# distributed-information-bottleneck/distributed-information-bottleneck.github.io

Measured on AMD Instinct MI355X. Metric: DIB train samples/sec (fwd+KL+bwd+Adam), higher is better.
Workload: dtype f32; 1 GPU; BASELINE config 3: synthetic tabular, 2^20 rows x 64 scalar features resident in HBM, posenc [2,4,8,16], encoder [128,128], E=32, integration [256,256], out=1, BCE-from-logits, Adam; per_gpu_batch=65536, global_batch=65536, parallelism=dp1, rccl_ranks_joined=1, dataset_rows=1048576, params=2224897

## Files before the change

### distributed-information-bottleneck.github.io_amd/_lib.py

```python
from __future__ import annotations

import ctypes
import os
import shutil
import subprocess
from ctypes import POINTER, c_char_p, c_float, c_int, c_int32, c_int64, c_uint32, c_uint64, c_void_p

_HERE = os.path.dirname(os.path.abspath(__file__))
CSRC = os.path.join(_HERE, "csrc")
LIB_PATH = os.path.join(_HERE, "libdib_hip.so")
LIB_OVERRIDE = os.environ.get("DIB_LIB_PATH") or None
INCLUDE_DIR = os.path.join(os.path.dirname(_HERE), "include")


def _sources() -> list:
    out = []
    for root, _, names in os.walk(CSRC):
        out += [os.path.join(root, n) for n in names if n.endswith((".h", ".hip"))]
    out += [os.path.join(INCLUDE_DIR, n) for n in os.listdir(INCLUDE_DIR) if n.endswith(".h")]
    return sorted(out)


DIB_OK = 0
ABI_VERSION = 7
# ... 85 lines not shown
    "dib_get_tuning": (c_int, [c_char_p, POINTER(c_int)]),
    "dib_adam_step": (c_int, [c_void_p, c_void_p, c_void_p, c_void_p, c_int64, c_void_p, c_void_p, c_float, c_float,
                              c_float, c_float, c_void_p]),
    "dib_sgd_step": (c_int, [c_void_p, c_void_p, c_int64, c_void_p, c_float, c_void_p]),
    "dib_encode_deterministic": (c_int, [c_void_p, c_int, c_void_p, c_int, c_void_p, c_void_p, c_void_p, c_void_p]),
    "dib_bhattacharyya": (c_int, [c_void_p, c_void_p, c_int, c_void_p, c_void_p, c_int, c_int, c_void_p, c_void_p]),
    "dib_infonce_workspace_bytes": (c_int64, [c_int]),
    "dib_infonce_fwd_bwd": (c_int, [c_void_p, c_void_p, c_int, c_int, c_int, c_float, c_void_p, c_void_p, c_void_p, c_void_p,
                                    c_void_p]),
    "dib_positional_encoding": (c_int, [c_void_p, c_int64, c_int, c_int, c_int, c_void_p, c_void_p]),
    "dib_positional_encoding_rows": (c_int, [c_void_p, c_int64, c_void_p, c_int, c_int, c_int, c_void_p, c_void_p]),
    "dib_mlp_small_supported": (c_int, [c_void_p, c_int]),
    "dib_mlp_small_fwd": (c_int, [c_void_p, c_void_p, c_void_p, c_int64, c_void_p, c_int, c_void_p, c_void_p, c_void_p, c_void_p]),
    "dib_mlp_small_bwd": (c_int, [c_void_p, c_void_p, c_void_p, c_void_p, c_void_p, c_int, c_void_p]),
    "dib_mlp_small_head_supported": (c_int, [c_void_p, c_int]),
    "dib_mlp_small_head_workspace_bytes": (c_int64, [c_void_p, c_int]),
    "dib_mlp_small_head_step": (c_int, [c_void_p, c_void_p, c_void_p, c_int, c_void_p, c_int64, c_int, c_float, c_void_p, c_void_p,
                                        c_void_p, c_void_p, c_void_p, c_void_p, c_void_p, c_void_p, c_void_p]),
    "dib_integration_fwd_and_mlp_fwd": (c_int, [c_void_p, c_int, c_void_p, c_void_p, c_void_p, c_void_p, c_void_p, c_int64, c_void_p,
                                                c_int, c_void_p, c_void_p, c_void_p, c_void_p]),
    "dib_backward_and_mlp_bwd": (c_int, [c_void_p, c_int, c_void_p, c_void_p, c_void_p, c_float, c_int, c_void_p, c_void_p, c_void_p,
                                         c_void_p, c_void_p, c_void_p, c_int, c_void_p]),
    "dib_reduce_adam_step": (c_int, [c_void_p, c_int, c_int64, c_void_p, c_void_p, c_void_p, c_void_p, c_int64, c_void_p, c_void_p,
                                     c_float, c_float, c_float, c_float, c_void_p, c_void_p]),
    "dib_mi_workspace_bytes": (c_int64, [c_int, c_int]),
    "dib_mi_sandwich_rows": (c_int, [c_void_p, c_int, c_int, c_uint64, c_uint32, c_uint32, c_void_p, c_void_p, c_void_p,
                                     c_void_p]),
    "dib_philox_normal_fill": (c_int, [c_void_p, c_void_p, c_int64, c_int, c_int, c_int, c_uint64, c_uint32,
                                       c_void_p]),
    "dib_philox_normal_ref": (c_float, [c_uint64, c_uint32, c_uint32, c_uint32, c_uint32]),
    "dib_launch_count": (c_int64, []),
    "dib_profile_enable": (c_int, [c_int]),
    "dib_profile_summary": (c_int, [POINTER(ctypes.c_double), POINTER(c_int)]),
    "dib_gemm": (c_int, [c_int, c_int, c_int, c_int, c_void_p, c_int, c_void_p, c_int, c_void_p, c_int, c_void_p,
                         c_void_p, c_int, c_int, c_void_p, c_void_p]),
}

SIGNATURES_ST = {
    "dib_gemm_grouped": (c_int, [c_int, c_int, c_void_p, c_int, c_int, c_void_p, c_void_p, c_void_p, c_void_p, c_void_p,
                                 c_void_p, c_int, c_int, c_int, c_int64, c_void_p]),
    "dib_reduce_splits": (c_int, [c_void_p, c_int64, c_int, c_int64, c_void_p, c_void_p]),
    "dib_reduce_splits_add": (c_int, [c_void_p, c_int64, c_int, c_int64, c_void_p, c_void_p]),
    "dib_gemm_skinny_k": (c_int, [c_int, c_int, c_void_p, c_int, c_int, c_int, c_void_p, c_void_p, c_void_p, c_void_p, c_void_p]),
    "dib_softmax_rows_fwd": (c_int, [c_void_p, c_int64, c_int, c_int, c_float, c_void_p]),
    "dib_softmax_rows_bwd": (c_int, [c_void_p, c_void_p, c_int64, c_int, c_int, c_float, c_void_p]),
    "dib_attention_stash_bytes": (c_int64, [c_int, c_int, c_int]),
    "dib_attention_fwd": (c_int, [c_void_p, c_void_p, c_void_p, c_int, c_int, c_int, c_int, c_int64, c_float, c_void_p, c_void_p,
                                  c_void_p, c_void_p]),
    "dib_attention_fwd_proj_supported": (c_int, [c_int, c_int, c_int]),
    "dib_attention_fwd_proj": (c_int, [c_void_p, c_int64, c_void_p, c_void_p, c_void_p, c_int, c_int, c_int, c_int, c_int, c_int64, c_float,
                                       c_void_p, c_void_p, c_void_p, c_void_p, c_void_p, c_void_p]),
    "dib_attention_bwd_proj": (c_int, [c_void_p, c_void_p, c_void_p, c_void_p, c_void_p, c_int, c_int, c_int, c_int, c_int, c_int64, c_float,
                                       c_void_p, c_void_p, c_void_p, c_void_p, c_void_p, c_void_p, c_int64, c_void_p]),
    "dib_attention_bwd_workspace_bytes": (c_int64, [c_int, c_int, c_int]),
    "dib_attention_bwd": (c_int, [c_void_p, c_void_p, c_void_p, c_void_p, c_void_p, c_void_p, c_void_p, c_int, c_int, c_int, c_int,
                                  c_int64, c_float, c_void_p, c_void_p, c_void_p, c_void_p, c_void_p]),
    "dib_add_layernorm_fwd": (c_int, [c_void_p, c_void_p, c_int, c_int64, c_int64, c_int, c_void_p, c_void_p, c_float, c_void_p,
                                      c_void_p, c_void_p, c_void_p]),
    "dib_add_layernorm_bwd_workspace_bytes": (c_int64, [c_int64, c_int]),
    "dib_add_layernorm_bwd": (c_int, [c_void_p, c_void_p, c_void_p, c_void_p, c_int64, c_int, c_void_p, c_void_p, c_void_p,
                                      c_void_p]),
    "dib_add_layernorm_bwd_fused": (c_int, [c_void_p, c_void_p, c_void_p, c_void_p, c_void_p, c_int64, c_int, c_void_p, c_void_p,
                                            c_int, c_void_p, c_void_p, c_void_p, c_void_p]),
    "dib_st_chain_supported": (c_int, [c_void_p, c_int64]),
    "dib_st_chain_workspace_bytes": (c_int64, [c_int64, c_int]),
    "dib_st_chain_fwd": (c_int, [c_void_p, c_int64, c_void_p, c_void_p, c_void_p, c_void_p, c_void_p, c_void_p, c_void_p, c_void_p,
                                 c_void_p, c_void_p, c_void_p]),
    "dib_st_chain_bwd": (c_int, [c_void_p, c_int64, c_void_p, c_void_p, c_int, c_int64, c_void_p, c_void_p, c_void_p, c_void_p, c_void_p,
                                 c_void_p, c_void_p, c_void_p, c_void_p, c_void_p, c_void_p]),
    "dib_mean_pool_fwd": (c_int, [c_void_p, c_int, c_int, c_int, c_void_p, c_void_p]),
    "dib_mean_pool_bwd": (c_int, [c_void_p, c_int, c_int, c_int, c_void_p, c_void_p]),
    "dib_add_inplace": (c_int, [c_void_p, c_void_p, c_int64, c_void_p]),
    "dib_act_grad_mul": (c_int, [c_void_p, c_void_p, c_int, c_int64, c_void_p, c_void_p]),
# ... 110 lines not shown
```

### distributed-information-bottleneck.github.io_amd/csrc/dib_api.hip

```cpp
#include <algorithm>
#include <atomic>
#include <cmath>
#include <cstdio>
#include <cstdlib>
#include <cstring>
#include <map>
#include <mutex>
#include <new>
#include <utility>
#include <vector>

#include "../../include/dib_hip.h"
#include "dib_elementwise.h"
#include "dib_gauss_lse.h"
#include "dib_mi_rows.h"
#include "dib_gemm.h"
#include "dib_infonce_mfma.h"
#include "dib_fused.h"
#include "dib_tail.h"
#include "dib_small.h"
#include "dib_st.h"
#include "dib_attn.h"
#include "dib_attn_small.h"
#include "dib_st_chain.h"
#include "dib_measure.h"
#include "dib_circuit.h"
#include "dib_partition.h"
#include "dib_st_info.h"
#include "dib_mi_channel.h"
#include "../../include/dib_st.h"
#include "../../include/dib_measure.h"
#include "../../include/dib_circuit.h"
#include "../../include/dib_partition.h"
#include "../../include/dib_mi_channel.h"

#include "host/common.h"
#include "host/layout.h"
#include "host/gemm.h"
#include "host/encoder.h"
#include "host/small.h"
#include "host/step.h"
#include "host/infonce.h"
#include "host/st.h"
#include "host/mi.h"
#include "host/measure.h"
#include "host/circuit.h"
#include "host/partition.h"
```

### distributed-information-bottleneck.github.io_amd/csrc/host/common.h

```cpp

static std::atomic<unsigned long long> g_dib_launches{0};
#define DIB_LAUNCH(...) do { g_dib_launches.fetch_add(1, std::memory_order_relaxed); hipLaunchKernelGGL(__VA_ARGS__); } while (0)

namespace {

constexpr int64_t kAlign = 64;
constexpr int kMaxSplits = 32;
constexpr int kSmallMaxBatch = 2048;
constexpr int kSmallMaxEncWgs = 1024;
constexpr size_t kSmallMaxLds = 160 * 1024;
constexpr int kSplitRows = 512;
inline int64_t align_up(int64_t v, int64_t a = kAlign) { return (v + a - 1) / a * a; }
inline int cdiv(int64_t a, int64_t b) { return (int)((a + b - 1) / b); }
inline int grid_for(int64_t n, int per_block = 256, int cap = 256 * 16) {
  return (int)std::max<int64_t>(1, std::min<int64_t>((n + per_block - 1) / per_block, cap));
}

constexpr int kProfCats = 17;
constexpr int kProfFusedFwd = 12, kProfFusedBwd = 13, kProfOther = 14, kProfAttnFwd = 15, kProfAttnBwd = 16;
struct Prof {
  std::atomic<bool> on{false};
  std::mutex mu;
  std::vector<hipEvent_t> pool;
  std::vector<std::pair<hipEvent_t, hipEvent_t>> spans[kProfCats];
  hipEvent_t get() {
    if (!pool.empty()) { hipEvent_t e = pool.back(); pool.pop_back(); return e; }
    hipEvent_t e = nullptr;
    (void)hipEventCreate(&e);
    return e;
  }
} g_prof;

struct ProfScope {
  int cat; hipStream_t st; hipEvent_t a = nullptr, b = nullptr;
  ProfScope(int c, hipStream_t s) : cat(c), st(s) {
    if (g_prof.on.load(std::memory_order_relaxed) && cat != 14) {
      { std::lock_guard<std::mutex> lk(g_prof.mu); a = g_prof.get(); b = g_prof.get(); }
      (void)hipEventRecord(a, st);
    }
  }
  ~ProfScope() {
    if (a) { (void)hipEventRecord(b, st); std::lock_guard<std::mutex> lk(g_prof.mu); g_prof.spans[cat].push_back({a, b}); }
  }
};

const char* kVersion = "dib_hip 0.4 (gfx950: fused encoder-bank fwd/bwd + grouped fp32-MFMA GEMM + flash attention)";

int act_ok(int a) { return a >= 0 && a <= 7; }

struct Tuning {
  int fwd_small_wgs = 512;
  int fwd_narrow_wgs = 1024;
  int stream_rows = 8192;
  int split_policy = 1;
  int split_overhead = 128;
  int fused_encoder = 1;
  int fused_head = 1;
  int small_batch = 1;
  int small_wgs = 512;
  int mlp_row_tiles = 1;
  int infonce_one_launch = 1;
  int attn_small_bwd_waves = 8;
  int wgrad_flat_tile = 1;
  int attn_fwd_waves = 8;
  int int_cluster_short_exchange = 1;
  int int_cluster = 8;
  int int_cluster_wgs = 256;
  int int_cluster_min_weights = 65536;
  int wgrad_max_splits = 32;
  int num_cus = 0;
};
inline Tuning& tuning() { static Tuning t; return t; }
inline const Tuning& knobs() { return tuning(); }
inline int wgrad_max_splits() { return std::max(1, std::min(32, knobs().wgrad_max_splits)); }
inline int device_cus() {
  static std::atomic<int> cus[64];
  int dev = 0;
  if (hipGetDevice(&dev) != hipSuccess || dev < 0 || dev >= 64) return 256;
  int v = cus[dev].load(std::memory_order_relaxed);
  if (v > 0) return v;
  if (hipDeviceGetAttribute(&v, hipDeviceAttributeMultiprocessorCount, dev) != hipSuccess || v <= 0) return 256;
  cus[dev].store(v, std::memory_order_relaxed);
  return v;
}
inline int split_rule_cus() { return knobs().num_cus > 0 ? knobs().num_cus : device_cus(); }

std::mutex g_attr_mu;
template <auto* Kernel>
int raise_dynamic_lds(size_t bytes) {
  if (bytes <= 64 * 1024) return DIB_OK;
  static std::atomic<size_t> granted[64];
  int dev = 0;
  std::atomic<size_t>* slot = hipGetDevice(&dev) == hipSuccess && dev >= 0 && dev < 64 ? &granted[dev] : nullptr;
  if (slot && slot->load(std::memory_order_acquire) >= bytes) return DIB_OK;
  std::lock_guard<std::mutex> lk(g_attr_mu);
  if (slot && slot->load(std::memory_order_relaxed) >= bytes) return DIB_OK;
  hipError_t e = hipFuncSetAttribute((const void*)Kernel, hipFuncAttributeMaxDynamicSharedMemorySize, (int)bytes);
  if (e != hipSuccess) return (int)e;
  if (slot) slot->store(bytes, std::memory_order_release);
  return DIB_OK;
}
template <auto* Kernel, typename... Args>
int launch_lds(dim3 grid, dim3 block, size_t lds, hipStream_t st, Args&&... args) {
  if (int rc = raise_dynamic_lds<Kernel>(lds)) return rc;
  DIB_LAUNCH(Kernel, grid, block, lds, st, std::forward<Args>(args)...);
  return (int)hipGetLastError();
}

static int* tuning_slot(const char* key) {
  Tuning& t = tuning();
  if (!key) return nullptr;
  if (!std::strcmp(key, "fwd_small_wgs")) return &t.fwd_small_wgs;
  if (!std::strcmp(key, "fwd_narrow_wgs")) return &t.fwd_narrow_wgs;
  if (!std::strcmp(key, "stream_rows")) return &t.stream_rows;
  if (!std::strcmp(key, "split_policy")) return &t.split_policy;
  if (!std::strcmp(key, "split_overhead")) return &t.split_overhead;
  if (!std::strcmp(key, "fused_encoder")) return &t.fused_encoder;
  if (!std::strcmp(key, "fused_head")) return &t.fused_head;
  if (!std::strcmp(key, "small_batch")) return &t.small_batch;
  if (!std::strcmp(key, "small_wgs")) return &t.small_wgs;
  if (!std::strcmp(key, "mlp_row_tiles")) return &t.mlp_row_tiles;
  if (!std::strcmp(key, "infonce_one_launch")) return &t.infonce_one_launch;
  if (!std::strcmp(key, "attn_small_bwd_waves")) return &t.attn_small_bwd_waves;
  if (!std::strcmp(key, "wgrad_flat_tile")) return &t.wgrad_flat_tile;
  if (!std::strcmp(key, "wgrad_max_splits")) return &t.wgrad_max_splits;
  if (!std::strcmp(key, "num_cus")) return &t.num_cus;
  if (!std::strcmp(key, "attn_fwd_waves")) return &t.attn_fwd_waves;
  if (!std::strcmp(key, "int_cluster_short_exchange")) return &t.int_cluster_short_exchange;
  if (!std::strcmp(key, "int_cluster")) return &t.int_cluster;
  if (!std::strcmp(key, "int_cluster_wgs")) return &t.int_cluster_wgs;
  if (!std::strcmp(key, "int_cluster_min_weights")) return &t.int_cluster_min_weights;
  return nullptr;
}

}

extern "C" {

const char* dib_version(void) { return kVersion; }
int dib_abi_version(void) { return DIB_ABI_VERSION; }

const char* dib_error_string(int code) {
  switch (code) {
    case DIB_OK: return "ok";
    case DIB_E_ARG: return "invalid argument";
    case DIB_E_SHAPE: return "shape mismatch";
    case DIB_E_WORKSPACE: return "workspace / descriptor tables missing";
    case DIB_E_UNSUPPORTED: return "unsupported configuration";
    case DIB_E_NODEVICE: return "no HIP device";
    default: return code > 0 ? hipGetErrorString((hipError_t)code) : "unknown dib error";
  }
}

int dib_set_tuning(const char* key, int value) {
  int* p = tuning_slot(key);
  if (!p || value < 0) return DIB_E_ARG;
  *p = value;
  return DIB_OK;
}

int dib_get_tuning(const char* key, int* value) {
  const int* p = tuning_slot(key);
  if (!p || !value) return DIB_E_ARG;
  *value = *p;
  return DIB_OK;
}

int64_t dib_launch_count(void) { return (int64_t)g_dib_launches.load(std::memory_order_relaxed); }

int dib_profile_enable(int on) {
  std::lock_guard<std::mutex> lk(g_prof.mu);
  for (int c = 0; c < kProfCats; ++c) {
    for (auto& sp : g_prof.spans[c]) { g_prof.pool.push_back(sp.first); g_prof.pool.push_back(sp.second); }
    g_prof.spans[c].clear();
  }
  g_prof.on = on != 0;
  return DIB_OK;
}

int dib_profile_summary(double* ms_by_category, int* launches_by_category) {
  if (!ms_by_category || !launches_by_category) return DIB_E_ARG;
  std::lock_guard<std::mutex> lk(g_prof.mu);
  for (int c = 0; c < kProfCats; ++c) {
    double tot = 0.0;
    for (auto& sp : g_prof.spans[c]) {
      hipError_t e = hipEventSynchronize(sp.second);
      if (e != hipSuccess) return (int)e;
      float ms = 0.f;
      e = hipEventElapsedTime(&ms, sp.first, sp.second);
      if (e != hipSuccess) return (int)e;
      tot += ms;
    }
    ms_by_category[c] = tot;
    launches_by_category[c] = (int)g_prof.spans[c].size();
  }
  return DIB_OK;
}

}
```

### distributed-information-bottleneck.github.io_amd/csrc/host/gemm.h

```cpp

namespace {

template <int MODE, int NI, int NJ, bool FLAT = false>
int launch_gemm_t(const DibGemmGroup* dev_groups, const GemmCall& c, int M, int N, const float* A, const float* B, float* C,
                  const float* bias, const float* aux, float* bias_out, int batch, int act, int nsplit,
                  int rows_per_split, long long split_stride, hipStream_t st) {
  const int tm = cdiv(M, FLAT ? 32 : 64 * NI), tn = cdiv(N, FLAT ? 256 : 64 * NJ);
  if (c.count > 65535 || (MODE == 2 && (long long)tm * tn > 65535)) return DIB_E_UNSUPPORTED;
  dim3 grid;
  if (MODE == 2) grid = dim3(nsplit, tm * tn, c.count);
  else grid = dim3(8 * cdiv(tm, 8) * tn, 1, c.count);
  constexpr int BK = FLAT ? 32 : ((NI == 2 && NJ == 2) ? 64 : ((MODE == 2 && NI == 1 && NJ == 2) ? 64 : 32));
  const long long streamed_rows = MODE == 2 ? (long long)nsplit * rows_per_split : (long long)M;
  const bool big_out = MODE != 2 && (long long)M * N * (long long)sizeof(float) * c.count >= (256ll << 20);
  const int stream_flags = streamed_rows >= knobs().stream_rows ? (big_out ? 3 : 1) : 0;
  DIB_LAUNCH((dib_gemm_kernel<MODE, NI, NJ, BK, FLAT>), grid, dim3(256), 0, st, dev_groups + c.first, A, B, C,
                     bias, aux, bias_out, batch, act, tm, tn, rows_per_split, split_stride, stream_flags);
  return (int)hipGetLastError();
}

static void pick_wgrad_splits(long long tiles, int slots, int K, int max_splits, int* ns_out, int* rps_out) {
  const int min_rows = std::min(kSplitRows, std::max(64, *rps_out));
  const auto cost_of = [&](int ns, int rps) {
    return (double)((tiles * ns + slots - 1) / slots) * (rps + knobs().split_overhead);
  };
  {
    const long long wgs = tiles * *ns_out, rounds = (wgs + slots - 1) / slots;
    if ((double)wgs >= 0.85 * (double)(rounds * slots)) return;
  }
  double best = 1e300;
  int bns = *ns_out, brps = *rps_out;
  for (int ns = 1; ns <= max_splits; ++ns) {
    const int rps = cdiv(cdiv(K, ns), 64) * 64;
    if (ns > 1 && rps < min_rows) break;
    if (cdiv(K, rps) != ns) continue;
    const double cost = cost_of(ns, rps);
    if (cost < best) {
      best = cost;
      bns = ns;
      brps = rps;
    }
  }
  if (best >= cost_of(*ns_out, *rps_out)) return;
  *ns_out = bns;
  *rps_out = brps;
}

template <int MODE>
int launch_gemm(const DibGemmGroup* dev_groups, const GemmCall& c, const float* A, const float* B, float* C,
                const float* bias, const float* aux, float* bias_out, int batch, int act, int nsplit, int rows_per_split,
                long long split_stride, hipStream_t st, bool auto_split = false, int max_splits = 0, int* ns_used = nullptr) {
  if (ns_used) *ns_used = nsplit;
  if (c.count == 0) return DIB_OK;
  const int M = c.max_m < 0 ? batch : c.max_m;
  const int N = c.max_n < 0 ? batch : c.max_n;
  bool ni1 = (MODE == 2) && M <= 64, nj1 = N <= 64;
  if (MODE != 2) {
    const long long wgs = (long long)cdiv(M, 128) * cdiv(N, nj1 ? 64 : 128) * c.count;
    if (wgs < knobs().fwd_small_wgs) ni1 = true;
    if (ni1 && !nj1 && (long long)cdiv(M, 64) * cdiv(N, 128) * c.count < (MODE == 0 ? knobs().fwd_narrow_wgs : 128)) nj1 = true;
  }
  if (MODE == 2 && !ni1 && !nj1) {
    const long long wgs = (long long)cdiv(M, 128) * cdiv(N, 128) * nsplit * c.count;
    if (wgs < 256) ni1 = true;
    if (ni1 && !nj1 && (long long)cdiv(M, 64) * cdiv(N, 128) * nsplit * c.count < 128) nj1 = true;
  }
  if (MODE == 2 && auto_split && nsplit > 1 && knobs().split_policy) {
    const int per_cu = (!ni1 && !nj1) ? 2 : ((!ni1 && nj1) ? 4 : (ni1 && !nj1) ? 3 : 4);
    const long long tiles = (long long)cdiv(M, ni1 ? 64 : 128) * cdiv(N, nj1 ? 64 : 128) * c.count;
    pick_wgrad_splits(tiles, split_rule_cus() * per_cu, batch, std::max(nsplit, max_splits), &nsplit, &rows_per_split);
    if (ns_used) *ns_used = nsplit;
  }
  ProfScope ps(MODE * 4 + (ni1 ? 0 : 2) + (nj1 ? 0 : 1), st);
  if constexpr (MODE == 2) {
    if (M <= 32 && N >= 256 && knobs().wgrad_flat_tile)
      return launch_gemm_t<2, 1, 2, true>(dev_groups, c, M, N, A, B, C, bias, aux, bias_out, batch, act, nsplit, rows_per_split,
                                          split_stride, st);
  }
#define DIB_GO(NI, NJ) launch_gemm_t<MODE, NI, NJ>(dev_groups, c, M, N, A, B, C, bias, aux, bias_out, batch, act, nsplit, \
                                                   rows_per_split, split_stride, st)
  if (ni1) return nj1 ? DIB_GO(1, 1) : DIB_GO(1, 2);
  return nj1 ? DIB_GO(2, 1) : DIB_GO(2, 2);
#undef DIB_GO
}

__global__ void dib_write_desc_kernel(DibGemmGroup* dst, DibGemmGroup g) { *dst = g; }

static int retire_stale_slabs(const dib_layout* l, int batch, const DibGemmGroup* host_groups, int count, int ns, int slab_count,
                              float* gt, long long split_stride, hipStream_t st) {
  hipStreamCaptureStatus cap = hipStreamCaptureStatusNone;
  const bool capturing = hipStreamIsCapturing(st, &cap) == hipSuccess && cap == hipStreamCaptureStatusActive;
  std::lock_guard<std::mutex> lk(l->wg_mu);
  for (int i = 0; i < count; ++i) {
    const DibGemmGroup& g = host_groups[i];
    int& mark = l->slab_hwm[std::make_pair(batch, g.c_off)];
    mark = std::max(mark, ns);
    const int hwm = capturing ? std::max(mark, slab_count) : mark;
    if (ns >= hwm) continue;
    const size_t wbytes = (size_t)g.M * (size_t)g.ldc * sizeof(float);
    for (int s = ns; s < hwm; ++s) {
      hipError_t e = hipMemsetAsync(gt + (long long)s * split_stride + g.c_off, 0, wbytes, st);
      if (e == hipSuccess && g.bias_off >= 0)
        e = hipMemsetAsync(gt + (long long)s * split_stride + g.bias_off, 0, (size_t)g.N * sizeof(float), st);
      if (e != hipSuccess) return (int)e;
    }
  }
  return DIB_OK;
}

template <int MODE>
int launch_gemm(const dib_layout* l, const GemmCall& c, const float* A, const float* B, float* C, const float* bias,
                const float* aux, float* bias_out, int batch, int act, int nsplit, int rows_per_split,
                long long split_stride, hipStream_t st, int slab_count = 0) {
  int ns_used = nsplit;
  int rc = launch_gemm<MODE>(l->dev_groups, c, A, B, C, bias, aux, bias_out, batch, act, nsplit, rows_per_split, split_stride,
                             st, MODE == 2, slab_count, &ns_used);
  if (MODE == 2 && rc == DIB_OK && slab_count > 1)
    rc = retire_stale_slabs(l, batch, l->table.data() + c.first, c.count, ns_used, slab_count, C, split_stride, st);
  return rc;
}

}

static int merged_wgrad(dib_layout* l, const dib_layout::WsMap& m, float* w, int batch, float* gt, int first, int count,
                        hipStream_t st) {
  if (count <= 0) return DIB_OK;
  const auto& host = wg_table_host(l, m, batch);
  GemmCall c;
  c.first = 0; c.count = count;
  for (int i = first; i < first + count; ++i) { c.max_m = std::max(c.max_m, host[i].M); c.max_n = std::max(c.max_n, host[i].N); }
  const DibGemmGroup* dev = reinterpret_cast<const DibGemmGroup*>(w + m.wg_table) + first;
  int ns_used = m.nsplit;
  int rc = launch_gemm<2>(dev, c, w, w, gt, nullptr, nullptr, gt, batch, 0, m.nsplit, m.rows_per_split, align_up(l->n_params, 4), st,
                          true, m.nsplit, &ns_used);
  if (rc == DIB_OK && m.nsplit > 1)
    rc = retire_stale_slabs(l, batch, host.data() + first, count, ns_used, m.nsplit, gt, align_up(l->n_params, 4), st);
  return rc;
}

extern "C" {

int dib_gemm(int mode, int M, int N, int K, const float* A, int lda, const float* B, int ldb, float* C, int ldc,
             const float* bias, const float* aux, int ldaux, int act, void* dev_desc, dib_stream_t stream) {
  if (!A || !B || !C || !dev_desc || M <= 0 || N <= 0 || K <= 0 || mode < 0 || mode > 2) return DIB_E_ARG;
  hipStream_t st = (hipStream_t)stream;
  DibGemmGroup g = make_group(Off(), lda, Off(), ldb, Off(), ldc, bias ? 0 : -1, Off(), ldaux, M, N, K);
  if ((((uintptr_t)A | (uintptr_t)B) & 15) != 0) return DIB_E_ARG;
  DIB_LAUNCH(dib_write_desc_kernel, dim3(1), dim3(1), 0, st, (DibGemmGroup*)dev_desc, g);
  if (hipError_t e = hipGetLastError(); e != hipSuccess) return (int)e;
  const int tm = cdiv(M, 128), tn = cdiv(N, 128);
  const DibGemmGroup* dg = (const DibGemmGroup*)dev_desc;
  const dim3 g1(8 * cdiv(tm, 8) * tn, 1, 1);
  if (mode == 0)
    DIB_LAUNCH((dib_gemm_kernel<0, 2, 2, 32>), g1, dim3(256), 0, st, dg, A, B, C, bias, aux, (float*)nullptr, 0,
                       act, tm, tn, 0, 0ll);
  else if (mode == 1)
    DIB_LAUNCH((dib_gemm_kernel<1, 2, 2, 32>), g1, dim3(256), 0, st, dg, A, B, C, bias, aux, (float*)nullptr, 0,
                       act, tm, tn, 0, 0ll);
  else
    DIB_LAUNCH((dib_gemm_kernel<2, 2, 2, 32>), dim3(1, tm * tn, 1), dim3(256), 0, st, dg, A, B, C,
                       (const float*)nullptr, aux, (float*)bias, 0, act, tm, tn, K, 0ll);
  return (int)hipGetLastError();
}

static_assert(sizeof(dib_gemm_desc) == sizeof(DibGemmGroup), "public descriptor must mirror the kernel's group struct");

int dib_gemm_grouped(int mode, int n_groups, const dib_gemm_desc* dev_desc, int max_m, int max_n, const float* A,
                     const float* B, float* C, const float* bias, const float* aux, float* bias_out, int act, int nsplit,
                     int rows_per_split, int64_t split_stride, dib_stream_t stream) {
  if (!dev_desc || !A || !B || !C || n_groups <= 0 || max_m <= 0 || max_n <= 0 || mode < 0 || mode > 2 || !act_ok(act))
    return DIB_E_ARG;
  if (mode == 2 && (nsplit <= 0 || rows_per_split <= 0)) return DIB_E_ARG;
  GemmCall c;
  c.first = 0; c.count = n_groups; c.max_m = max_m; c.max_n = max_n;
  const DibGemmGroup* g = reinterpret_cast<const DibGemmGroup*>(dev_desc);
  hipStream_t st = (hipStream_t)stream;
  switch (mode) {
    case 0: return launch_gemm<0>(g, c, A, B, C, bias, aux, nullptr, 0, act, 1, 0, 0, st);
    case 1: return launch_gemm<1>(g, c, A, B, C, nullptr, aux, nullptr, 0, act, 1, 0, 0, st);
    default: return launch_gemm<2>(g, c, A, B, C, nullptr, nullptr, bias_out, 0, 0, nsplit, rows_per_split,
                                   (long long)split_stride, st);
  }
}

int dib_gemm_skinny_k(int mode, int n_groups, const dib_gemm_desc* dev_desc, int M, int N, int K, const float* A,
                      const float* B, float* C, const float* bias, dib_stream_t stream) {
  if (!dev_desc || !A || !B || !C || n_groups <= 0 || M <= 0 || N <= 0 || K <= 0 || mode < 0 || mode > 1) return DIB_E_ARG;
  if (K > 32 || (K & 3) || (N & 31) || n_groups > 65535 || cdiv(N, 128) > 65535) return DIB_E_UNSUPPORTED;
  const DibGemmGroup* g = reinterpret_cast<const DibGemmGroup*>(dev_desc);
  const int total_tiles = cdiv(M, 64), cn = cdiv(N, 128);
  int chunks = std::max(1, std::min(total_tiles, cdiv(4096, cn * n_groups)));
  int tiles = std::min(8, cdiv(total_tiles, chunks));
  chunks = cdiv(total_tiles, tiles);
  const int nt_store = (long long)M * N * (long long)sizeof(float) * n_groups >= (256ll << 20) ? 1 : 0;
  const dim3 grid(chunks, cn, n_groups);
  hipStream_t st = (hipStream_t)stream;
  if (mode == 0)
    DIB_LAUNCH(dib_gemm_skinnyk_kernel<0>, grid, dim3(256), 0, st, g, A, B, C, bias, M, N, K, tiles, nt_store);
  else
    DIB_LAUNCH(dib_gemm_skinnyk_kernel<1>, grid, dim3(256), 0, st, g, A, B, C, (const float*)nullptr, M, N, K, tiles,
                       nt_store);
  return (int)hipGetLastError();
}

int dib_reduce_splits(const float* partial, int64_t n, int nsplit, int64_t stride, float* out, dib_stream_t stream) {
  if (!partial || !out || n <= 0 || nsplit <= 0 || (n & 3) || (stride & 3)) return DIB_E_ARG;
  DIB_LAUNCH(dib_reduce_splits_kernel, dim3(grid_for(n / 4)), dim3(256), 0, (hipStream_t)stream, partial,
                     (long long)n, nsplit, (long long)stride, out, (const float*)nullptr);
  return (int)hipGetLastError();
}

int dib_reduce_splits_add(const float* partial, int64_t n, int nsplit, int64_t stride, float* out, dib_stream_t stream) {
  if (!partial || !out || n <= 0 || nsplit <= 0 || (n & 3) || (stride & 3)) return DIB_E_ARG;
  DIB_LAUNCH(dib_reduce_splits_kernel, dim3(grid_for(n / 4)), dim3(256), 0, (hipStream_t)stream, partial,
                     (long long)n, nsplit, (long long)stride, out, (const float*)out);
  return (int)hipGetLastError();
}
// ... 3 lines not shown
```

### distributed-information-bottleneck.github.io_amd/engine.py

```python
from __future__ import annotations

import ctypes
import math
from ctypes import byref, c_int, c_int64, c_void_p
from typing import Dict, List, Optional, Sequence

import numpy as np
import torch

from . import _lib
from ._lib import ACTIVATIONS, LOSS_KINDS, check
from .utils import mi_sandwich_rows


def _ptr(t: Optional[torch.Tensor]):
    return c_void_p(t.data_ptr()) if t is not None else c_void_p(0)


class HipEngine:

    def __init__(self, feature_dimensionalities: Sequence[int], feature_encoder_architecture: Sequence[int],
                 integration_network_architecture: Sequence[int], output_dimensionality: int,
                 use_positional_encoding: bool = True, number_positional_encoding_frequencies: int = 5,
                 activation_fn: Optional[str] = "relu", feature_embedding_dimension: int = 32,
# ... 442 lines not shown
        assert loss.numel() == 1 and loss.dtype == torch.float32 and loss.device == self.device
        gx = gy = None
        if want_grads:
            for o in (out_gx, out_gy):
                assert o is None or (o.is_contiguous() and tuple(o.shape) == (b, d) and o.dtype == torch.float32)
            gx = out_gx if out_gx is not None else torch.empty_like(emb_x)
            gy = out_gy if out_gy is not None else torch.empty_like(emb_y)
        check(self.lib.dib_infonce_fwd_bwd(_ptr(emb_x), _ptr(emb_y), b, d, _lib.SIMILARITIES[similarity], float(temperature),
                                           _ptr(gx), _ptr(gy), _ptr(loss), _ptr(ws), self._stream()), "dib_infonce_fwd_bwd")
        return loss, gx, gy

    def backward_from_pred_grad(self, g_pred: torch.Tensor, row_idx, row0: int, batch: int, seed: int, step: int,
                                inv_global_batch: Optional[float] = None, finish_flags: int = 0, optimizer=None,
                                companion=None, metrics_acc: Optional[torch.Tensor] = None) -> None:
        inv = 1.0 / batch if inv_global_batch is None else inv_global_batch
        dst = self.g_pred(batch)
        if not (g_pred.data_ptr() == dst.data_ptr() and g_pred.shape == dst.shape and g_pred.stride() == dst.stride()):
            dst.copy_(g_pred)
        self.backward(row_idx, row0, batch, seed, step, inv, finish_flags=finish_flags, optimizer=optimizer, companion=companion,
                      metrics_acc=metrics_acc)

    def mi_sandwich_bounds(self, enc_out: torch.Tensor, seed: int, step: int, feature: int):
        rows = mi_sandwich_rows(self.lib, self.device, self.to_device(enc_out), seed, step, feature)
        m = rows.mean(dim=1).cpu().numpy()
        return float(m[0]), float(m[1])

    def eps(self, row_idx, row0: int, batch: int, seed: int, step: int) -> torch.Tensor:
        out = torch.empty((batch, self.F, self.E), dtype=torch.float32, device=self.device)
        check(self.lib.dib_philox_normal_fill(_ptr(out), _ptr(row_idx), int(row0), batch, self.F, self.E, int(seed),
                                              int(step) & 0xFFFFFFFF, self._stream()), "dib_philox_normal_fill")
        return out


PROFILE_CATEGORIES = 17


def profile_summary(lib) -> dict:
    ms = (ctypes.c_double * PROFILE_CATEGORIES)()
    cnt = (c_int * PROFILE_CATEGORIES)()
    check(lib.dib_profile_summary(ms, cnt), "dib_profile_summary")
    bk = lambda mode, ni, nj: 64 if (ni, nj) == (2, 2) or (mode, ni, nj) == (2, 1, 2) else 32
    names = [f"dib_gemm_kernel<{mode}, {ni}, {nj}, {bk(mode, ni, nj)}>"
             for mode in (0, 1, 2) for ni in (1, 2) for nj in (1, 2)]
    names += ["dib_fused_encoder_fwd_kernel", "dib_fused_encoder_bwd_kernel", "other", "dib_attn_fwd_kernel", "dib_attn_bwd_kernel"]
    return {n: (float(ms[i]), int(cnt[i])) for i, n in enumerate(names) if cnt[i]}
```

### include/dib_hip.h

```cpp
#ifndef DIB_HIP_H
#define DIB_HIP_H

#include <stdint.h>

#ifdef __cplusplus
extern "C" {
#endif

typedef struct dib_layout dib_layout;
typedef void* dib_stream_t;

#define DIB_OK 0
#define DIB_E_ARG (-1)
#define DIB_E_SHAPE (-2)
#define DIB_E_WORKSPACE (-3)
#define DIB_E_UNSUPPORTED (-4)
#define DIB_E_NODEVICE (-5)

enum { DIB_ACT_LINEAR = 0, DIB_ACT_RELU = 1, DIB_ACT_LEAKY_RELU = 2, DIB_ACT_TANH = 3,
       DIB_ACT_SIGMOID = 4, DIB_ACT_ELU = 5, DIB_ACT_SOFTPLUS = 6 };

enum { DIB_LOSS_BCE_LOGITS = 0, DIB_LOSS_BCE = 1, DIB_LOSS_SPARSE_CCE_LOGITS = 2, DIB_LOSS_MSE = 3 };

enum { DIB_WS_U = 0,
// ... 102 lines not shown
typedef struct dib_mlp_desc {
  int64_t w_off[4], b_off[4];
  int32_t n_hidden, width[4];
  int32_t in_dim, n_freq, act;
} dib_mlp_desc;
int dib_mlp_small_supported(const dib_mlp_desc* d, int batch);
int dib_mlp_small_fwd(const dib_mlp_desc* d, const float* params, const float* x, int64_t ldx, const int32_t* row_idx, int n,
                      float* a0, float* const* h, float* out, dib_stream_t stream);
int dib_mlp_small_bwd(const dib_mlp_desc* d, const float* params, const float* g_out, float* const* h, float* const* g, int n,
                      dib_stream_t stream);
int dib_mlp_small_head_supported(const dib_mlp_desc* d, int n);
int64_t dib_mlp_small_head_workspace_bytes(const dib_mlp_desc* d, int n);
int dib_mlp_small_head_step(const dib_mlp_desc* d, const float* params, const float* x, int n, const float* y, int64_t ldy,
                            int loss_kind, float inv_global_batch, float* const* h, float* const* g, float* pred, float* g_pred,
                            float* g_x, float* grads, float* sums3, void* ws, dib_stream_t stream);
int dib_integration_fwd_and_mlp_fwd(dib_layout* l, int batch, const float* params, void* ws, const dib_mlp_desc* d,
                                    const float* mlp_params, const float* x, int64_t ldx, const int32_t* row_idx, int n, float* a0,
                                    float* const* h, float* out, dib_stream_t stream);
int dib_backward_and_mlp_bwd(dib_layout* l, int batch, const float* params, float* grads, const float* beta_dev,
                             float inv_global_batch, int flags, void* ws, const dib_mlp_desc* d, const float* mlp_params,
                             const float* g_out, float* const* h, float* const* g, int n, dib_stream_t stream);

int64_t dib_mi_workspace_bytes(int n, int embedding_dim);
int dib_mi_sandwich_rows(const float* enc_out, int n, int embedding_dim, uint64_t seed, uint32_t step,
                         uint32_t feature, double* lower_rows, double* upper_rows, void* ws, dib_stream_t stream);
int dib_philox_normal_fill(float* eps, const int32_t* row_idx, int64_t row0, int batch, int num_features,
                           int embedding_dim, uint64_t seed, uint32_t step, dib_stream_t stream);
float dib_philox_normal_ref(uint64_t seed, uint32_t step, uint32_t row, uint32_t feature, uint32_t e);

int64_t dib_launch_count(void);
#define DIB_PROFILE_CATEGORIES 17
int dib_profile_enable(int on);
int dib_profile_summary(double* ms_by_category , int* launches_by_category );

int dib_gemm(int mode, int M, int N, int K, const float* A, int lda, const float* B, int ldb, float* C,
             int ldc, const float* bias, const float* aux, int ldaux, int act, void* dev_desc ,
             dib_stream_t stream);

#ifdef __cplusplus
}
#endif
#endif
```

### include/dib_st.h

```cpp
#ifndef DIB_ST_H
#define DIB_ST_H
#include "dib_hip.h"

#ifdef __cplusplus
extern "C" {
#endif

#define DIB_ACT_LEAKY_RELU_01 7

typedef struct dib_gemm_desc {
  int64_t a_off, b_off, c_off, bias_off, aux_off;
  int64_t a_boff, b_boff, c_boff, aux_boff;
  int32_t M, N, K;
  int32_t lda, ldb, ldc, ldaux;
  int32_t flags;
} dib_gemm_desc;

int dib_gemm_grouped(int mode, int n_groups, const dib_gemm_desc* dev_desc, int max_m, int max_n, const float* A,
                     const float* B, float* C, const float* bias, const float* aux, float* bias_out, int act, int nsplit,
                     int rows_per_split, int64_t split_stride, dib_stream_t stream);
int dib_reduce_splits(const float* partial, int64_t n, int nsplit, int64_t stride, float* out, dib_stream_t stream);
int dib_reduce_splits_add(const float* partial, int64_t n, int nsplit, int64_t stride, float* out, dib_stream_t stream);

int dib_gemm_skinny_k(int mode, int n_groups, const dib_gemm_desc* dev_desc, int M, int N, int K, const float* A,
                      const float* B, float* C, const float* bias, dib_stream_t stream);

int dib_softmax_rows_fwd(float* S, int64_t rows, int P, int ld, float scale, dib_stream_t stream);
int dib_softmax_rows_bwd(const float* P_probs, float* dP, int64_t rows, int P, int ld, float scale, dib_stream_t stream);

int64_t dib_attention_stash_bytes(int B, int P, int H);
int dib_attention_fwd(const float* q, const float* k, const float* v, int B, int P, int H, int key_dim, int64_t ld,
                      float scale, float* o, float* lse, float* s_stash, dib_stream_t stream);
int64_t dib_attention_bwd_workspace_bytes(int B, int P, int H);
int dib_attention_fwd_proj_supported(int P, int key_dim, int model_dim);
int dib_attention_fwd_proj(const float* x, int64_t ldx, const float* params, const int64_t* w_off, const int64_t* b_off, int B, int P,
                           int H, int key_dim, int model_dim, int64_t ld, float scale, float* q, float* k, float* v, float* o,
                           float* lse, dib_stream_t stream);
int dib_attention_bwd_proj(const float* q, const float* k, const float* v, const float* d_o, const float* lse, int B, int P, int H,
                           int key_dim, int model_dim, int64_t ld, float scale, float* dq, float* dk, float* dv, const float* params,
                           const int64_t* w_off, float* dx_slabs, int64_t slab_stride, dib_stream_t stream);
int dib_attention_bwd(const float* q, const float* k, const float* v, const float* o, const float* d_o, const float* lse,
                      const float* s_stash, int B, int P, int H, int key_dim, int64_t ld, float scale, float* dq, float* dk,
                      float* dv, void* ws, dib_stream_t stream);

int dib_add_layernorm_fwd(const float* a, const float* b, int b_slabs, int64_t b_stride, int64_t T, int D, const float* gamma,
                          const float* beta, float eps, float* y, float* xhat, float* rstd, dib_stream_t stream);
int64_t dib_add_layernorm_bwd_workspace_bytes(int64_t T, int D);
int dib_add_layernorm_bwd(const float* dy, const float* xhat, const float* rstd, const float* gamma, int64_t T, int D,
                          float* ds, float* dgamma_dbeta, void* ws, dib_stream_t stream);
typedef struct dib_st_block_desc {
  int64_t o_w, o_b, ln1_g, ln1_b, ln2_g, ln2_b, ff_w[3], ff_b[3];
  int32_t n_ff, ff_width[3];
  int32_t D, HK;
// ... 50 lines not shown
```

Baseline: 8.362 million samples/s.

## Add register-streamed MFMA weight-gradient kernel with fused bias reduction

Adds a new weight-gradient GEMM kernel in which each wave owns a 128-column output tile and streams A/B rows straight from global memory through a four-deep register ring, prefetching ahead of the MFMA work. It folds the bias-gradient column sum into the same pass using cross-half lane shuffles. The kernel replaces the LDS-tiled wgrad path when shapes, alignment and slab occupancy checks pass, and can use nontemporal loads for long K. The aim is to cut LDS staging and sync overhead on tall-K wgrad GEMMs, in exchange for heavy register pressure (one wave per SIMD) and reliance on latency hiding through prefetch alone. Profiling categories and a host-side API entry are extended to cover it.

```diff
diff --git a/distributed-information-bottleneck.github.io_amd/_lib.py b/distributed-information-bottleneck.github.io_amd/_lib.py
--- a/distributed-information-bottleneck.github.io_amd/_lib.py
+++ b/distributed-information-bottleneck.github.io_amd/_lib.py
@@ -141,6 +141,7 @@
     "dib_launch_count": (c_int64, []),
     "dib_profile_enable": (c_int, [c_int]),
     "dib_profile_summary": (c_int, [POINTER(ctypes.c_double), POINTER(c_int)]),
+    "dib_profile_summary_n": (c_int, [POINTER(ctypes.c_double), POINTER(c_int), c_int]),
     "dib_gemm": (c_int, [c_int, c_int, c_int, c_int, c_void_p, c_int, c_void_p, c_int, c_void_p, c_int, c_void_p,
                          c_void_p, c_int, c_int, c_void_p, c_void_p]),
 }
@@ -148,6 +149,8 @@
 SIGNATURES_ST = {
     "dib_gemm_grouped": (c_int, [c_int, c_int, c_void_p, c_int, c_int, c_void_p, c_void_p, c_void_p, c_void_p, c_void_p,
                                  c_void_p, c_int, c_int, c_int, c_int64, c_void_p]),
+    "dib_wgrad_grouped": (c_int, [c_int, c_void_p, c_void_p, c_int, c_int, c_int, c_void_p, c_void_p, c_void_p, c_void_p, c_int,
+                                  c_int, c_int64, c_void_p]),
     "dib_reduce_splits": (c_int, [c_void_p, c_int64, c_int, c_int64, c_void_p, c_void_p]),
     "dib_reduce_splits_add": (c_int, [c_void_p, c_int64, c_int, c_int64, c_void_p, c_void_p]),
     "dib_gemm_skinny_k": (c_int, [c_int, c_int, c_void_p, c_int, c_int, c_int, c_void_p, c_void_p, c_void_p, c_void_p, c_void_p]),
diff --git a/distributed-information-bottleneck.github.io_amd/csrc/dib_api.hip b/distributed-information-bottleneck.github.io_amd/csrc/dib_api.hip
--- a/distributed-information-bottleneck.github.io_amd/csrc/dib_api.hip
+++ b/distributed-information-bottleneck.github.io_amd/csrc/dib_api.hip
@@ -15,6 +15,7 @@
 #include "dib_gauss_lse.h"
 #include "dib_mi_rows.h"
 #include "dib_gemm.h"
+#include "dib_wgrad_stream.h"
 #include "dib_infonce_mfma.h"
 #include "dib_fused.h"
 #include "dib_tail.h"
diff --git a/distributed-information-bottleneck.github.io_amd/csrc/dib_wgrad_stream.h b/distributed-information-bottleneck.github.io_amd/csrc/dib_wgrad_stream.h
--- /dev/null
+++ b/distributed-information-bottleneck.github.io_amd/csrc/dib_wgrad_stream.h
@@ -0,0 +1,134 @@
+#pragma once
+#include "dib_gemm.h"
+
+constexpr int kWgsGroups = 4;
+constexpr int kWgsRing = 4 * kWgsGroups;
+
+__device__ __forceinline__ float dib_wgs_swap_halves(float v) { return __shfl_xor(v, 32, 64); }
+
+template <int NT, int CH, bool NTL>
+__global__ void __launch_bounds__(256, 1)
+dib_wgrad_stream_kernel(const DibGemmGroup* __restrict__ groups, const float* __restrict__ Abase,
+                        const float* __restrict__ Bbase, float* __restrict__ Cbase, float* __restrict__ bias_out, int batch,
+                        int count, int tiles_m, int tiles_n, int nsplit, int rows_per_split, long long split_stride) {
+  static_assert((NT == 4 && (CH == 2 || CH == 4)) || (NT == 2 && CH == 4), "128- or 64-column tiles; the tiled kernels' bias chains");
+  static_assert(kWgsGroups == 4, "the bias chains below are laid out for a ring of four 8-row blocks");
+  constexpr int G = kWgsGroups;
+  typedef float f4v __attribute__((ext_vector_type(4)));
+  typedef float fbv __attribute__((ext_vector_type(NT)));
+  const int lane = threadIdx.x & 63, l31 = lane & 31, h = lane >> 5;
+  const int wave = __builtin_amdgcn_readfirstlane((int)(threadIdx.x >> 6));
+  const unsigned wid = blockIdx.x * 4u + (unsigned)wave;
+  const unsigned tiles = (unsigned)(tiles_m * tiles_n);
+  if (wid >= tiles * (unsigned)count * (unsigned)nsplit) return;
+  const int tile = (int)(wid % tiles);
+  const int grp = (int)((wid / tiles) % (unsigned)count), slab = (int)(wid / (tiles * (unsigned)count));
+  const int tm = tile / tiles_n, tn = tile % tiles_n;
+  const DibGemmGroup g = groups[grp];
+  const int M = g.M < 0 ? batch : g.M;
+  const int N = g.N < 0 ? batch : g.N;
+  const int K = g.K < 0 ? batch : g.K;
+  const int m0 = tm * 128, n0 = tn * (32 * NT);
+  if (m0 >= M || n0 >= N) return;
+  const int kbeg = slab * rows_per_split;
+  const int nblk = max(0, min(K, kbeg + rows_per_split) - kbeg) >> 3;
+
+  const char* pA = reinterpret_cast<const char*>(Abase + g.a_off + g.a_boff * batch + (long long)(kbeg + 4 * h) * g.lda + m0 + 4 * l31);
+  const char* pB = reinterpret_cast<const char*>(Bbase + g.b_off + g.b_boff * batch + (long long)(kbeg + 4 * h) * g.ldb + n0 + NT * l31);
+  const unsigned rowA = (unsigned)g.lda * 4u, rowB = (unsigned)g.ldb * 4u;
+
+  dib_f32x16 acc[4][NT];
+#pragma unroll
+  for (int i = 0; i < 4; ++i)
+#pragma unroll
+    for (int j = 0; j < NT; ++j)
+#pragma unroll
+      for (int r = 0; r < 16; ++r) acc[i][j][r] = 0.f;
+
+  fbv x[CH];
+#pragma unroll
+  for (int c = 0; c < CH; ++c) x[c] = 0.f;
+
+  f4v ra[G][4];
+  fbv rb[G][4];
+  auto load_step = [&](int slot, int blk, int t) {
+    const f4v* pa = reinterpret_cast<const f4v*>(pA + (size_t)((unsigned)(8 * blk + t) * rowA));
+    const fbv* pb = reinterpret_cast<const fbv*>(pB + (size_t)((unsigned)(8 * blk + t) * rowB));
+    if (NTL) {
+      ra[slot][t] = __builtin_nontemporal_load(pa);
+      rb[slot][t] = __builtin_nontemporal_load(pb);
+    } else {
+      ra[slot][t] = *pa;
+      rb[slot][t] = *pb;
+    }
+  };
+  if (nblk > 0) {
+#pragma unroll
+    for (int j = 0; j < G - 1; ++j)
+#pragma unroll
+      for (int t = 0; t < 4; ++t) load_step(j, j, t);
+  }
+#pragma unroll 1
+  for (int q0 = 0; q0 < nblk; q0 += G) {
+#pragma unroll
+    for (int j = 0; j < G; ++j) {
+      const int pf = min(q0 + j + G - 1, nblk - 1);
+#pragma unroll
+      for (int t = 0; t < 4; ++t) {
+        const f4v a = ra[j][t];
+        const fbv b = rb[j][t];
+#pragma unroll
+        for (int i = 0; i < 4; ++i)
+#pragma unroll
+          for (int u = 0; u < NT; ++u) acc[i][u] = DIB_MFMA(a[i], b[u], acc[i][u]);
+        __builtin_amdgcn_sched_barrier(0);
+        load_step((j + G - 1) % G, pf, t);
+        __builtin_amdgcn_sched_barrier(0);
+      }
+      fbv& xc = x[CH == 2 ? 0 : j];
+      fbv y = xc;
+#pragma unroll
+      for (int t = 0; t < 4; ++t) y += rb[j][t];
+#pragma unroll
+      for (int u = 0; u < NT; ++u) y[u] = dib_wgs_swap_halves(y[u]);
+#pragma unroll
+      for (int t = 0; t < 4; ++t) y += rb[j][t];
+#pragma unroll
+      for (int u = 0; u < NT; ++u) xc[u] = dib_wgs_swap_halves(y[u]);
+    }
+    if (CH == 2) {
+      const fbv s = x[0];
+      x[0] = x[1];
+      x[1] = s;
+    }
+  }
+
+  const long long coff = g.c_off + g.c_boff * batch + (long long)slab * split_stride;
+  float* Cg = Cbase + coff;
+  const bool vecC = ((coff | (long long)g.ldc) & (NT - 1)) == 0;
+#pragma unroll
+  for (int i = 0; i < 4; ++i) {
+#pragma unroll
+    for (int r = 0; r < 16; ++r) {
+      const int m = m0 + 4 * ((r & 3) + 8 * (r >> 2) + 4 * h) + i;
+      float* cp = Cg + (long long)m * g.ldc + n0 + NT * l31;
+      fbv v;
+#pragma unroll
+      for (int u = 0; u < NT; ++u) v[u] = acc[i][u][r];
+      if (vecC) {
+        *reinterpret_cast<fbv*>(cp) = v;
+      } else {
+#pragma unroll
+        for (int u = 0; u < NT; ++u) cp[u] = v[u];
+      }
+    }
+  }
+  if (bias_out != nullptr && g.bias_off >= 0 && tm == 0 && h == 0) {
+    fbv s = x[0];
+#pragma unroll
+    for (int c = 1; c < CH; ++c) s += x[c];
+    float* bp = bias_out + g.bias_off + (long long)slab * split_stride + n0 + NT * l31;
+#pragma unroll
+    for (int u = 0; u < NT; ++u) bp[u] = s[u];
+  }
+}
diff --git a/distributed-information-bottleneck.github.io_amd/csrc/host/common.h b/distributed-information-bottleneck.github.io_amd/csrc/host/common.h
--- a/distributed-information-bottleneck.github.io_amd/csrc/host/common.h
+++ b/distributed-information-bottleneck.github.io_amd/csrc/host/common.h
@@ -16,8 +16,9 @@
   return (int)std::max<int64_t>(1, std::min<int64_t>((n + per_block - 1) / per_block, cap));
 }
 
-constexpr int kProfCats = 17;
+constexpr int kProfCats = 19;
 constexpr int kProfFusedFwd = 12, kProfFusedBwd = 13, kProfOther = 14, kProfAttnFwd = 15, kProfAttnBwd = 16;
+constexpr int kProfWgradStream128 = 17, kProfWgradStream64 = 18;
 struct Prof {
   std::atomic<bool> on{false};
   std::mutex mu;
@@ -62,6 +63,9 @@
   int infonce_one_launch = 1;
   int attn_small_bwd_waves = 8;
   int wgrad_flat_tile = 1;
+  int wgrad_stream = 1;
+  int wgrad_stream_rows = 8192;
+  int wgrad_stream_fill = 85;
   int attn_fwd_waves = 8;
   int int_cluster_short_exchange = 1;
   int int_cluster = 8;
@@ -123,6 +127,9 @@
   if (!std::strcmp(key, "infonce_one_launch")) return &t.infonce_one_launch;
   if (!std::strcmp(key, "attn_small_bwd_waves")) return &t.attn_small_bwd_waves;
   if (!std::strcmp(key, "wgrad_flat_tile")) return &t.wgrad_flat_tile;
+  if (!std::strcmp(key, "wgrad_stream")) return &t.wgrad_stream;
+  if (!std::strcmp(key, "wgrad_stream_rows")) return &t.wgrad_stream_rows;
+  if (!std::strcmp(key, "wgrad_stream_fill")) return &t.wgrad_stream_fill;
   if (!std::strcmp(key, "wgrad_max_splits")) return &t.wgrad_max_splits;
   if (!std::strcmp(key, "num_cus")) return &t.num_cus;
   if (!std::strcmp(key, "attn_fwd_waves")) return &t.attn_fwd_waves;
@@ -178,10 +185,10 @@
   return DIB_OK;
 }
 
-int dib_profile_summary(double* ms_by_category, int* launches_by_category) {
-  if (!ms_by_category || !launches_by_category) return DIB_E_ARG;
+int dib_profile_summary_n(double* ms_by_category, int* launches_by_category, int n) {
+  if (!ms_by_category || !launches_by_category || n < 0) return DIB_E_ARG;
   std::lock_guard<std::mutex> lk(g_prof.mu);
-  for (int c = 0; c < kProfCats; ++c) {
+  for (int c = 0; c < std::min(n, kProfCats); ++c) {
     double tot = 0.0;
     for (auto& sp : g_prof.spans[c]) {
       hipError_t e = hipEventSynchronize(sp.second);
@@ -194,7 +201,12 @@
     ms_by_category[c] = tot;
     launches_by_category[c] = (int)g_prof.spans[c].size();
   }
-  return DIB_OK;
-}
-
-}
+  for (int c = kProfCats; c < n; ++c) { ms_by_category[c] = 0.0; launches_by_category[c] = 0; }
+  return DIB_OK;
+}
+
+int dib_profile_summary(double* ms_by_category, int* launches_by_category) {
+  return dib_profile_summary_n(ms_by_category, launches_by_category, DIB_PROFILE_CATEGORIES);
+}
+
+}
diff --git a/distributed-information-bottleneck.github.io_amd/csrc/host/gemm.h b/distributed-information-bottleneck.github.io_amd/csrc/host/gemm.h
--- a/distributed-information-bottleneck.github.io_amd/csrc/host/gemm.h
+++ b/distributed-information-bottleneck.github.io_amd/csrc/host/gemm.h
@@ -19,6 +19,51 @@
   return (int)hipGetLastError();
 }
 
+constexpr int kWgradStreamWavesPerCu = 4;
+static bool wgrad_stream_shape_ok(const DibGemmGroup* hg, int count, int batch, const float* A, const float* B, int* nt_out) {
+  if (!knobs().wgrad_stream || !hg || count <= 0) return false;
+  if ((((uintptr_t)A | (uintptr_t)B) & 15) != 0) return false;
+  int nt = 0;
+  for (int i = 0; i < count; ++i) {
+    const DibGemmGroup& g = hg[i];
+    const int M = g.M < 0 ? batch : g.M, N = g.N < 0 ? batch : g.N, K = g.K < 0 ? batch : g.K;
+    if (M <= 0 || (M & 127) || K <= 0 || (K & 63)) return false;
+    const int nt_g = N == 64 ? 2 : ((N > 0 && (N & 127) == 0) ? 4 : 0);
+    if (!nt_g || (nt && nt != nt_g)) return false;
+    nt = nt_g;
+    if (((g.a_off + g.a_boff * batch) | (g.b_off + g.b_boff * batch) | (long long)g.lda | (long long)g.ldb) & 3) return false;
+    if (g.lda < M || g.ldb < N) return false;
+  }
+  *nt_out = nt;
+  return true;
+}
+static bool wgrad_stream_slabs_ok(const DibGemmGroup* hg, int count, int batch, long long tiles, int nsplit, int rows_per_split) {
+  if (nsplit <= 0 || rows_per_split <= 0 || (long long)nsplit * rows_per_split < knobs().wgrad_stream_rows) return false;
+  if (tiles * nsplit * 100 < (long long)knobs().wgrad_stream_fill * split_rule_cus() * kWgradStreamWavesPerCu) return false;
+  for (int i = 0; i < count; ++i) {
+    const int K = hg[i].K < 0 ? batch : hg[i].K;
+    if ((rows_per_split & 63) && !(nsplit == 1 && rows_per_split >= K)) return false;
+    if (((long long)std::min(rows_per_split, K) + 8) * std::max(hg[i].lda, hg[i].ldb) * 4 >= (1ll << 31)) return false;
+  }
+  return true;
+}
+template <int NT, int CH>
+int launch_wgrad_stream(const DibGemmGroup* dev_groups, const GemmCall& c, int M, int N, const float* A, const float* B, float* C,
+                        float* bias_out, int batch, int nsplit, int rows_per_split, long long split_stride, hipStream_t st) {
+  const int tm = cdiv(M, 128), tn = cdiv(N, 32 * NT);
+  const long long waves = (long long)tm * tn * c.count * nsplit;
+  if (waves >= (1ll << 31)) return DIB_E_UNSUPPORTED;
+  ProfScope ps(NT == 4 ? kProfWgradStream128 : kProfWgradStream64, st);
+  const dim3 grid((unsigned)((waves + 3) / 4));
+  if ((long long)nsplit * rows_per_split >= knobs().stream_rows)
+    DIB_LAUNCH((dib_wgrad_stream_kernel<NT, CH, true>), grid, dim3(256), 0, st, dev_groups + c.first, A, B, C, bias_out, batch,
+               c.count, tm, tn, nsplit, rows_per_split, split_stride);
+  else
+    DIB_LAUNCH((dib_wgrad_stream_kernel<NT, CH, false>), grid, dim3(256), 0, st, dev_groups + c.first, A, B, C, bias_out, batch,
+               c.count, tm, tn, nsplit, rows_per_split, split_stride);
+  return (int)hipGetLastError();
+}
+
 static void pick_wgrad_splits(long long tiles, int slots, int K, int max_splits, int* ns_out, int* rps_out) {
   const int min_rows = std::min(kSplitRows, std::max(64, *rps_out));
   const auto cost_of = [&](int ns, int rps) {
@@ -49,7 +94,8 @@
 template <int MODE>
 int launch_gemm(const DibGemmGroup* dev_groups, const GemmCall& c, const float* A, const float* B, float* C,
                 const float* bias, const float* aux, float* bias_out, int batch, int act, int nsplit, int rows_per_split,
-                long long split_stride, hipStream_t st, bool auto_split = false, int max_splits = 0, int* ns_used = nullptr) {
+                long long split_stride, hipStream_t st, bool auto_split = false, int max_splits = 0, int* ns_used = nullptr,
+                const DibGemmGroup* host_groups = nullptr) {
   if (ns_used) *ns_used = nsplit;
   if (c.count == 0) return DIB_OK;
   const int M = c.max_m < 0 ? batch : c.max_m;
@@ -64,6 +110,21 @@
     const long long wgs = (long long)cdiv(M, 128) * cdiv(N, 128) * nsplit * c.count;
     if (wgs < 256) ni1 = true;
     if (ni1 && !nj1 && (long long)cdiv(M, 64) * cdiv(N, 128) * nsplit * c.count < 128) nj1 = true;
+  }
+  if constexpr (MODE == 2) {
+    int nt = 0;
+    if (wgrad_stream_shape_ok(host_groups, c.count, batch, A, B, &nt)) {
+      int ns = nsplit, rps = rows_per_split;
+      const long long tiles = (long long)cdiv(M, 128) * cdiv(N, 32 * nt) * c.count;
+      if (auto_split && ns > 1 && knobs().split_policy)
+        pick_wgrad_splits(tiles, split_rule_cus() * kWgradStreamWavesPerCu, batch, std::max(ns, max_splits), &ns, &rps);
+      if (wgrad_stream_slabs_ok(host_groups, c.count, batch, tiles, ns, rps)) {
+        if (ns_used) *ns_used = ns;
+        if (nt == 2) return launch_wgrad_stream<2, 4>(dev_groups, c, M, N, A, B, C, bias_out, batch, ns, rps, split_stride, st);
+        return nj1 ? launch_wgrad_stream<4, 4>(dev_groups, c, M, N, A, B, C, bias_out, batch, ns, rps, split_stride, st)
+                   : launch_wgrad_stream<4, 2>(dev_groups, c, M, N, A, B, C, bias_out, batch, ns, rps, split_stride, st);
+      }
+    }
   }
   if (MODE == 2 && auto_split && nsplit > 1 && knobs().split_policy) {
     const int per_cu = (!ni1 && !nj1) ? 2 : ((!ni1 && nj1) ? 4 : (ni1 && !nj1) ? 3 : 4);
@@ -114,7 +175,7 @@
                 long long split_stride, hipStream_t st, int slab_count = 0) {
   int ns_used = nsplit;
   int rc = launch_gemm<MODE>(l->dev_groups, c, A, B, C, bias, aux, bias_out, batch, act, nsplit, rows_per_split, split_stride,
-                             st, MODE == 2, slab_count, &ns_used);
+                             st, MODE == 2, slab_count, &ns_used, MODE == 2 ? l->table.data() + c.first : nullptr);
   if (MODE == 2 && rc == DIB_OK && slab_count > 1)
     rc = retire_stale_slabs(l, batch, l->table.data() + c.first, c.count, ns_used, slab_count, C, split_stride, st);
   return rc;
@@ -132,7 +193,7 @@
   const DibGemmGroup* dev = reinterpret_cast<const DibGemmGroup*>(w + m.wg_table) + first;
   int ns_used = m.nsplit;
   int rc = launch_gemm<2>(dev, c, w, w, gt, nullptr, nullptr, gt, batch, 0, m.nsplit, m.rows_per_split, align_up(l->n_params, 4), st,
-                          true, m.nsplit, &ns_used);
+                          true, m.nsplit, &ns_used, host.data() + first);
   if (rc == DIB_OK && m.nsplit > 1)
     rc = retire_stale_slabs(l, batch, host.data() + first, count, ns_used, m.nsplit, gt, align_up(l->n_params, 4), st);
   return rc;
@@ -183,6 +244,19 @@
   }
 }
 
+int dib_wgrad_grouped(int n_groups, const dib_gemm_desc* dev_desc, const dib_gemm_desc* host_desc, int max_m, int max_n, int batch,
+                      const float* A, const float* B, float* C, float* bias_out, int nsplit, int rows_per_split,
+                      int64_t split_stride, dib_stream_t stream) {
+  if (!dev_desc || !host_desc || !A || !B || !C || n_groups <= 0 || max_m <= 0 || max_n <= 0 || batch < 0 || nsplit <= 0 ||
+      rows_per_split <= 0)
+    return DIB_E_ARG;
+  GemmCall c;
+  c.first = 0; c.count = n_groups; c.max_m = max_m; c.max_n = max_n;
+  return launch_gemm<2>(reinterpret_cast<const DibGemmGroup*>(dev_desc), c, A, B, C, nullptr, nullptr, bias_out, batch, 0, nsplit,
+                        rows_per_split, (long long)split_stride, (hipStream_t)stream, false, 0, nullptr,
+                        reinterpret_cast<const DibGemmGroup*>(host_desc));
+}
+
 int dib_gemm_skinny_k(int mode, int n_groups, const dib_gemm_desc* dev_desc, int M, int N, int K, const float* A,
                       const float* B, float* C, const float* bias, dib_stream_t stream) {
   if (!dev_desc || !A || !B || !C || n_groups <= 0 || M <= 0 || N <= 0 || K <= 0 || mode < 0 || mode > 1) return DIB_E_ARG;
diff --git a/distributed-information-bottleneck.github.io_amd/engine.py b/distributed-information-bottleneck.github.io_amd/engine.py
--- a/distributed-information-bottleneck.github.io_amd/engine.py
+++ b/distributed-information-bottleneck.github.io_amd/engine.py
@@ -498,15 +498,16 @@
         return out
 
 
-PROFILE_CATEGORIES = 17
+PROFILE_CATEGORIES = 19
 
 
 def profile_summary(lib) -> dict:
     ms = (ctypes.c_double * PROFILE_CATEGORIES)()
     cnt = (c_int * PROFILE_CATEGORIES)()
-    check(lib.dib_profile_summary(ms, cnt), "dib_profile_summary")
+    check(lib.dib_profile_summary_n(ms, cnt, PROFILE_CATEGORIES), "dib_profile_summary_n")
     bk = lambda mode, ni, nj: 64 if (ni, nj) == (2, 2) or (mode, ni, nj) == (2, 1, 2) else 32
     names = [f"dib_gemm_kernel<{mode}, {ni}, {nj}, {bk(mode, ni, nj)}>"
              for mode in (0, 1, 2) for ni in (1, 2) for nj in (1, 2)]
     names += ["dib_fused_encoder_fwd_kernel", "dib_fused_encoder_bwd_kernel", "other", "dib_attn_fwd_kernel", "dib_attn_bwd_kernel"]
+    names += ["dib_wgrad_stream_kernel<4>", "dib_wgrad_stream_kernel<2>"]
     return {n: (float(ms[i]), int(cnt[i])) for i, n in enumerate(names) if cnt[i]}
diff --git a/include/dib_hip.h b/include/dib_hip.h
--- a/include/dib_hip.h
+++ b/include/dib_hip.h
@@ -158,6 +158,8 @@
 #define DIB_PROFILE_CATEGORIES 17
 int dib_profile_enable(int on);
 int dib_profile_summary(double* ms_by_category , int* launches_by_category );
+#define DIB_PROFILE_CATEGORIES_N 19
+int dib_profile_summary_n(double* ms_by_category , int* launches_by_category , int n);
 
 int dib_gemm(int mode, int M, int N, int K, const float* A, int lda, const float* B, int ldb, float* C,
              int ldc, const float* bias, const float* aux, int ldaux, int act, void* dev_desc ,
diff --git a/include/dib_st.h b/include/dib_st.h
--- a/include/dib_st.h
+++ b/include/dib_st.h
@@ -19,6 +19,9 @@
 int dib_gemm_grouped(int mode, int n_groups, const dib_gemm_desc* dev_desc, int max_m, int max_n, const float* A,
                      const float* B, float* C, const float* bias, const float* aux, float* bias_out, int act, int nsplit,
                      int rows_per_split, int64_t split_stride, dib_stream_t stream);
+int dib_wgrad_grouped(int n_groups, const dib_gemm_desc* dev_desc, const dib_gemm_desc* host_desc, int max_m, int max_n,
+                      int batch, const float* A, const float* B, float* C, float* bias_out, int nsplit, int rows_per_split,
+                      int64_t split_stride, dib_stream_t stream);
 int dib_reduce_splits(const float* partial, int64_t n, int nsplit, int64_t stride, float* out, dib_stream_t stream);
 int dib_reduce_splits_add(const float* partial, int64_t n, int nsplit, int64_t stride, float* out, dib_stream_t stream);
 
```

After: 8.493 million samples/s, median of 6. 1.02x the previous value.
